# bharatlytics/faceRecognition_InfrenceEngine

Hardware: AMD Instinct MI355X
Metric: faces/sec end-to-end @1080p (higher is better)
Workload: dtype f16

## Files before the change

facerecognition_infrenceengine_amd/_lib.py:

```python
import ctypes as C
import struct
import os
import threading

_HERE = os.path.dirname(os.path.abspath(__file__))
LIB_PATH = os.path.join(_HERE, "csrc", "libfrhip.so")

_lock = threading.Lock()
_lib = None
ABI_VERSION = 104


class FrError(RuntimeError):
    pass


class ConvArgs(C.Structure):
    _fields_ = [("x", C.c_void_p), ("w", C.c_void_p), ("y", C.c_void_p),
                ("bias", C.c_void_p), ("slope", C.c_void_p), ("residual", C.c_void_p),
                ("out_f32_partial", C.c_void_p),
                ("B", C.c_int), ("H", C.c_int), ("W", C.c_int), ("Cin", C.c_int), ("Cout", C.c_int),
                ("KH", C.c_int), ("KW", C.c_int), ("stride", C.c_int), ("pad", C.c_int),
                ("Ho", C.c_int), ("Wo", C.c_int), ("bias_mode", C.c_int), ("splitk", C.c_int),
                ("x2", C.c_void_p), ("C2", C.c_int)]


class ConvStep(C.Structure):
    _fields_ = [("kind", C.c_int), ("args", ConvArgs)]


class ConvF8Args(C.Structure):
    _fields_ = [("x8", C.c_void_p), ("w8", C.c_void_p), ("y16", C.c_void_p), ("y8", C.c_void_p),
                ("oscale", C.c_void_p), ("bias", C.c_void_p), ("slope", C.c_void_p), ("residual", C.c_void_p),
                ("B", C.c_int), ("H", C.c_int), ("W", C.c_int), ("Cin", C.c_int), ("Cout", C.c_int),
                ("bias_mode", C.c_int), ("y8_mul", C.c_float), ("y8_sub", C.c_void_p)]


class RolePtr(C.c_void_p):
    role = None


class PnetLevel(C.Structure):
    _fields_ = [("x1", C.c_void_p), ("head", C.c_void_p), ("workspace", C.c_void_p), ("H1", C.c_int), ("W1", C.c_int),
# ... 50 lines not shown
    "fr_conv_walk64_weight_bytes": (_Z, [_I]),
    "fr_conv_walk64_pack": (_I, [_P, _P, _I, _P]),
    "fr_conv_walk64_f16": (_I, [_P, _P, _P, _P, _I, _P, _P, _I, _I, _I, _P]),
    "fr_conv_stage28_weight_bytes": (_Z, [_I]),
    "fr_conv_stage28_pack": (_I, [_P, _P, _P]),
    "fr_conv_stage28_f16": (_I, [_P, _P, _P, _P, _I, _I, _P]),
    "fr_conv_stage14_f8_weight_bytes": (_Z, [_I]),
    "fr_conv_stage14_f8_param_floats": (_Z, []),
    "fr_conv_stage14_f8_pack": (_I, [_P, _P, _P]),
    "fr_conv_stage14_f8": (_I, [_P, _P, _P, _P, _P, _I, _I, _P]),
    "fr_conv_splitk_epilogue": (_I, [_P, _I, _I, _I, _I, _I, _P, _I, _P, _P, _P, _P]),
    "fr_fc_reduce_l2norm": (_I, [_P, _I, _I, _I, _P, _P, _P, _P]),
    "fr_warp_affine_5pt": (_I, [_P, _I, _I, _I, _P, _P, _P, _I, _I, _P, _P, _P, _P]),
    "fr_warp_affine_5pt_slots": (_I, [_P, _I, _I, _I, _P, _P, _I, _I, _P, _P]),
    "fr_pyramid_resize_norm": (_I, [_P, _I, _I, _I, _I, _I, _P, _P]),
    "fr_dconv_f32": (_I, [_P, _P, _P, _P, _P, _I, _I, _I, _I, _I, _I, _I, _I, _I, _P, _P, _I, _P]),
    "fr_dconv_mfma_f32": (_I, [_I, _P, _P, _P, _P, _P, _I, _I, _I, _P, _P, _P, _I, _I, _P, _I, _P, _P]),
    "fr_crop_conv1_f32": (_I, [_I, _P, _I, _I, _I, _P, _P, _I, _P, _P, _P, _P, _P]),
    "fr_crop_conv1_split": (_I, [_I, _P, _I, _I, _I, _P, _P, _I, _P, _P, _P, _P, _I, _P]),
    "fr_crop_conv1_list_f32": (_I, [_I, _P, _I, _I, _I, _P, _I, _P, _P, _I, _P, _P, _P, _P, _P]),
    "fr_ro_conv2_split": (_I, [_I, _P, _P, _P, _P, _P, _I, _P, _I, _P, _P]),
    "fr_ro_gemm_weight_bytes": (_Z, [_I]),
    "fr_ro_gemm_pack": (_I, [_I, _P, _P, _P]),
    "fr_ro_gemm_split": (_I, [_I, _P, _P, _P, _P, _P, _I, _P, _I, _P]),
    "fr_ro_margin_list": (_I, [_P, _I, _P, _I, _I, _F, _F, _P, _P, _I, _P]),
    "fr_ro_scatter_rows": (_I, [_P, _P, _P, _I, _I, _P, _P]),
    "fr_pnet23_workspace_bytes": (_Z, [_I, _I, _I]),
    "fr_pnet23_split_f16": (_I, [_P, _P, _I, _I, _I, _P, _P, _P, _P, _P, _P, _P, _P, _P, _I, _F, _F, _P, _P, _Z, _P]),
    "fr_maxpool_f32": (_I, [_P, _P, _I, _I, _I, _I, _I, _I, _P]),
    "fr_pnet_conv1_band": (_I, [_I, _P, _I, _I, _I, _I, _I, _P, _P, _P, _P, _P, _P, _P, _I, _P]),
    "fr_pnet_band_tiles_count": (_Z, [_I, _I, _I]),
    "fr_pnet_band_tiles": (_I, [_P, _I, _I, _I, _P, _P, _P]),
    "fr_pnet_finish_levels": (_I, [C.POINTER(PnetLevel), _I, _I, _P, _P, _P, _P, _P, _P, _P, _P, _F, _I, _F, _P, _P]),
    "fr_pnet_pyramid_conv1": (_I, [_I, _P, _I, _I, _I, C.POINTER(PnetLevel), _I, _P, _P, _P, _P, _P, _I, _P]),
    "fr_pnet_pyramid_p23": (_I, [C.POINTER(PnetLevel), _I, _I, _P, _P, _P, _P, _P, _P, _P, _P, _I, _F, _F, _P]),
    "fr_pnet_pyramid_band_tiles": (_I, [C.POINTER(PnetLevel), _I, _I, _P, _P, _P]),
    "fr_pnet_candidates": (_I, [_P, _I, _I, _I, _F, _F, _I, _P, _P, _P, _P, _P, _P, _P, _F, _P]),
    "fr_sort_nms": (_I, [_P, _P, _P, _I, _P, _I, _I, _I, _I, _F, _I, _I, _P, _P, _P, _P, _I, _P]),
    "fr_box_refine": (_I, [_P, _P, _I, _P, _I, _I, _I, _P]),
    "fr_crop_resize_norm": (_I, [_P, _I, _I, _I, _P, _P, _I, _I, _P, _P]),
    "fr_stage_select": (_I, [_P, _P, _I, _P, _I, _I, _F, _P, _P, _P, _I, _P, _P, _P]),
    "fr_detect_sequence": (_I, [C.POINTER(Call), _I]),
}

_NOCHECK = ("fr_version", "fr_device_count")


def _slot(v, t):
    if t is _F:
        return struct.unpack("<I", struct.pack("<f", float(v)))[0]
    if t is _P:
        if v is None:
            return 0
        return int(v.value or 0) if isinstance(v, C.c_void_p) else int(v)
    return int(v) & 0xFFFFFFFFFFFFFFFF


class Lib:

    def __init__(self, cdll):
        self._c = cdll
        self._calls = {}
        self._rec = threading.local()
        for name, (res, args) in SIGNATURES.items():
            fn = getattr(cdll, name)
            fn.restype = res
# ... 91 lines not shown
```

facerecognition_infrenceengine_amd/csrc/detect_ops.hip:

```cpp
#include "detect_math.h"

__global__ void pyramid_resize_norm(const uint8_t* __restrict__ frames, int N, int H, int W, int hs, int ws,
                                    float* __restrict__ out) {
    int64_t t = (int64_t)blockIdx.x * blockDim.x + threadIdx.x;
    int64_t total = (int64_t)N * hs * ws;
    if (t >= total) return;
    int x = (int)(t % ws);
    int y = (int)((t / ws) % hs);
    int n = (int)(t / ((int64_t)ws * hs));
    const float ry = (float)H / (float)hs, rx = (float)W / (float)ws;
    Lerp ly = lerp_coord(y, ry, H), lx = lerp_coord(x, rx, W);
    const uint8_t* f = frames + (int64_t)n * H * W * 3;
    const uint8_t* r0 = f + (int64_t)ly.i0 * W * 3;
    const uint8_t* r1 = f + (int64_t)ly.i1 * W * 3;
    float* o = out + t * 3;
#pragma unroll
    for (int c = 0; c < 3; ++c) {
        int ci = 2 - c;
        float v = bilerp((float)r0[lx.i0 * 3 + ci], (float)r0[lx.i1 * 3 + ci], (float)r1[lx.i0 * 3 + ci],
                         (float)r1[lx.i1 * 3 + ci], lx.w, ly.w);
        o[c] = (v - 127.5f) * 0.0078125f;
    }
}

// ... 260 lines not shown
    const int cell = b * 256 + threadIdx.x;
    bool pass = false;
    float p = 0.f;
    const float* h = t.head[l] + ((int64_t)f * cells + (cell < cells ? cell : 0)) * 6;
    if (cell < cells && dl_may_pass(t.dl[l][(int64_t)f * cells + cell], dl_min)) {
        p = softmax2_face(h[0], h[1]);
        pass = p >= thr;
    }
    const int lane = threadIdx.x & 63, wv = threadIdx.x >> 6;
    unsigned long long m = __ballot(pass);
    if (lane == 0) wsum[wv] = __popcll(m);
    __syncthreads();
    int woff = 0;
    for (int i = 0; i < wv; ++i) woff += wsum[i];
    const int rank = base + woff + __popcll(m & ((1ull << lane) - 1ull));
    if (pass && rank < cap) {
        const int cy = cell / wc, cx = cell - cy * wc;
        const int64_t o = (int64_t)f * cap + rank;
        float4 bx;
        bx.x = floorf((2.0f * (float)cx + 1.0f) / scale);
        bx.y = floorf((2.0f * (float)cy + 1.0f) / scale);
        bx.z = floorf((2.0f * (float)cx + 12.0f) / scale);
        bx.w = floorf((2.0f * (float)cy + 12.0f) / scale);
        *reinterpret_cast<float4*>(t.boxes[l] + o * 4) = bx;
        t.scores[l][o] = p;
        *reinterpret_cast<float4*>(t.regs[l] + o * 4) = make_float4(h[2], h[3], h[4], h[5]);
    }
    if (b == nb - 1 && threadIdx.x == 0) {
        int total = base + wsum[0] + wsum[1] + wsum[2] + wsum[3];
        t.counts[l][f] = total < cap ? total : cap;
    }
}

int fr_pnet_candidates_levels_launch(const fr_pnet_level* lv, int nlevels, int nframes, float thr, int cap, float dl_min, hipStream_t s) {
    PCandLevels t;
    t.nlevels = nlevels;
    int total = 0;
    for (int l = 0; l < nlevels; ++l) {
        const int hc = lv[l].H1 - 4, wc = lv[l].W1 - 4;
        t.head[l] = lv[l].head; t.dl[l] = reinterpret_cast<const float*>(lv[l].workspace);
        t.boxes[l] = lv[l].boxes; t.scores[l] = lv[l].scores; t.regs[l] = lv[l].regs; t.counts[l] = lv[l].counts;
        t.block_counts[l] = lv[l].block_counts;
        t.cells[l] = hc * wc; t.wc[l] = wc; t.scale[l] = lv[l].scale;
        t.first[l] = total;
        total += fr_cdiv(hc * wc, 256);
    }
    t.first[nlevels] = total;
    dim3 grid(total, nframes);
    pnet_count_levels<<<grid, 256, 0, s>>>(t, thr, dl_min);
    FR_CHECK_LAUNCH("pnet_count_levels");
    pnet_emit_levels<<<grid, 256, 0, s>>>(t, thr, cap, dl_min);
    FR_CHECK_LAUNCH("pnet_emit_levels");
    return FR_OK;
}

extern "C" int fr_pnet_candidates(const float* head, int nframes, int hc, int wc, float scale, float thr, int cap,
                                  float* boxes, float* scores, float* regs, int32_t* counts, int32_t* block_counts,
                                  float* prob_out, const float* dl, float dl_min, fr_stream_t stream) {
    FR_REQUIRE(head && boxes && scores && regs && counts && block_counts, "fr_pnet_candidates: null pointer");
    FR_REQUIRE(nframes > 0 && hc > 0 && wc > 0 && cap > 0 && scale > 0.f, "fr_pnet_candidates: bad argument");
    const int cells = hc * wc;
    dim3 grid(fr_cdiv(cells, 256), nframes);
    hipStream_t s = fr_stream(stream);
    pnet_count<<<grid, 256, 0, s>>>(head, cells, thr, block_counts, prob_out, dl, dl_min);
    FR_CHECK_LAUNCH("pnet_count");
    pnet_emit<<<grid, 256, 0, s>>>(head, cells, wc, scale, thr, cap, block_counts, boxes, scores, regs, counts, dl, dl_min);
    FR_CHECK_LAUNCH("pnet_emit");
    return FR_OK;
}

__global__ void box_refine(float* __restrict__ boxes, const float* __restrict__ aux, int naux,
                           const int32_t* __restrict__ counts, int L, int cap, int mode) {
    int t = blockIdx.x * blockDim.x + threadIdx.x;
    if (t >= L * cap) return;
    int l = t / cap, i = t - l * cap;
    if (i >= counts[l]) return;
    float4 b = *reinterpret_cast<float4*>(boxes + (int64_t)t * 4);
    const float* r = aux + (int64_t)t * naux;
    float add = mode == 0 ? 0.0f : 1.0f;
    float w = b.z - b.x + add, h = b.w - b.y + add;
    float x1 = b.x + r[0] * w, y1 = b.y + r[1] * h, x2 = b.z + r[2] * w, y2 = b.w + r[3] * h;
    if (mode != 2) {
        float hh = y2 - y1, ww = x2 - x1;
        float l2 = fmaxf(ww, hh);
        x1 = x1 + ww * 0.5f - l2 * 0.5f;
        y1 = y1 + hh * 0.5f - l2 * 0.5f;
// ... 141 lines not shown
```

facerecognition_infrenceengine_amd/csrc/pnet_fused.hip:

```cpp
#include "detect_math.h"

#define P23_RH 8
#define P23_RW 32
#define P23_X1W (P23_RW + 4)
#define P23_X1PX ((P23_RH + 4) * P23_X1W)
#define P23_X2W (P23_RW + 2)
#define P23_X2PX ((P23_RH + 2) * P23_X2W)
#define P23_X2T ((P23_X2PX + 15) / 16)
#define P23_NT 512
#define P23_X1PL (448 * 32)
#define P23_X2PL (P23_X2PX * 32)

struct P23Args {
    const float* x1;
    const unsigned char* x1s;
    unsigned x1s_bytes;
    const float* w2; const float* b2; const float* s2;
    const float* w3; const float* b3; const float* s3;
    const float* hw; const float* hb;
    float* head;
    float* dl;
    int all_heads;
    int* list; int* counts; int seg_cap;
    float logit_thr;
// ... 384 lines not shown
    P23Args a;
    a.x1 = x1; a.x1s = (const unsigned char*)x1s; a.x1s_bytes = (unsigned)((int64_t)B * H1 * W1 * 64); a.w2 = w2; a.b2 = b2; a.s2 = s2; a.w3 = w3; a.b3 = b3; a.s3 = s3; a.hw = hw; a.hb = hb; a.head = head; a.all_heads = all_heads & 1;
    a.B = B; a.H1 = H1; a.W1 = W1; a.H3 = H1 - 4; a.W3 = W1 - 4;
    a.tiles_x = (a.W3 + P23_RW - 1) / P23_RW; a.tiles_y = (a.H3 + P23_RH - 1) / P23_RH;
    long long ncell, nt; int grid, seg_cap;
    p23_layout(B, H1, W1, ncell, nt, grid, seg_cap);
    FR_REQUIRE(nt < (1ll << 31) && ncell < (1ll << 31), "fr_pnet23_split_f16: too many tiles");
    const size_t need = fr_pnet23_workspace_bytes(B, H1, W1);
    FR_REQUIRE(workspace && workspace_bytes >= need, "fr_pnet23_split_f16: workspace needs %zu bytes (fr_pnet23_workspace_bytes)", need);
    a.dl = reinterpret_cast<float*>(workspace);
    a.counts = reinterpret_cast<int*>(a.dl + ncell);
    a.list = a.counts + 512;
    a.seg_cap = seg_cap;
    a.logit_thr = refine_logit_thr;
    a.band_hi = refine_band_hi;
    a.ntiles = (int)nt;
    constexpr size_t lds = (size_t)2 * P23_X1PL + (size_t)2 * P23_X2PL + 30 * 1024 + 108 * 4;
    static FrDevLatch latch;
    if (!fr_raise_lds(reinterpret_cast<const void*>(pnet23_split_f16), lds, latch)) { fr_set_error("fr_pnet23_split_f16: cannot raise dynamic LDS"); return FR_E_LAUNCH; }
    hipStream_t s = fr_stream(stream);
    pnet23_split_f16<<<grid, P23_NT, lds, s>>>(a);
    FR_CHECK_LAUNCH("pnet23_split_f16");
    if (all_heads & 2) return FR_OK;
    PRefArgs r;
    r.x1 = x1; r.w2 = w2; r.b2 = b2; r.s2 = s2; r.w3 = w3; r.b3 = b3; r.s3 = s3; r.hw = hw; r.hb = hb; r.head = head;
    r.list = a.list; r.counts = a.counts; r.seg_cap = seg_cap;
    r.B = B; r.H1 = H1; r.W1 = W1; r.H3 = a.H3; r.W3 = a.W3; r.counter = refined_count;
    pnet_refine_mfma<<<grid, 256, 0, s>>>(r);
    FR_CHECK_LAUNCH("pnet_refine_mfma");
    return FR_OK;
}

int fr_pnet_candidates_levels_launch(const fr_pnet_level* lv, int nlevels, int nframes, float thr, int cap, float dl_min, hipStream_t s);

extern "C" int fr_pnet_finish_levels(const fr_pnet_level* levels, int nlevels, int nframes, const float* w2, const float* b2,
                                     const float* s2, const float* w3, const float* b3, const float* s3, const float* hw,
                                     const float* hb, float thr, int cap, float dl_min, int32_t* refined_count, fr_stream_t stream) {
    FR_REQUIRE(levels && nlevels > 0 && nlevels <= PREF_MAXL && nframes > 0 && cap > 0, "fr_pnet_finish_levels: 1 .. %d levels", PREF_MAXL);
    FR_REQUIRE(w2 && b2 && s2 && w3 && b3 && s3 && hw && hb, "fr_pnet_finish_levels: null pointer");
    PRefLevels t;
    t.nlevels = nlevels;
    int total = 0;
    for (int l = 0; l < nlevels; ++l) {
        const fr_pnet_level& L = levels[l];
        FR_REQUIRE(L.x1 && L.head && L.workspace && L.boxes && L.scores && L.regs && L.counts && L.block_counts && L.H1 >= 5 && L.W1 >= 5 && L.scale > 0.f,
                   "fr_pnet_finish_levels: level %d: bad entry", l);
        long long ncell, nt; int grid, seg_cap;
        p23_layout(nframes, L.H1, L.W1, ncell, nt, grid, seg_cap);
        float* dl = reinterpret_cast<float*>(L.workspace);
        const int* counts = reinterpret_cast<const int*>(dl + ncell);
        t.x1[l] = L.x1; t.head[l] = L.head; t.counts[l] = counts; t.list[l] = counts + 512;
        t.seg_cap[l] = seg_cap; t.H1[l] = L.H1; t.W1[l] = L.W1;
        t.first[l] = total;
        total += grid;
    }
    t.first[nlevels] = total;
    PRefArgs r;
    r.x1 = nullptr; r.w2 = w2; r.b2 = b2; r.s2 = s2; r.w3 = w3; r.b3 = b3; r.s3 = s3; r.hw = hw; r.hb = hb; r.head = nullptr;
    r.list = nullptr; r.counts = nullptr; r.seg_cap = 0; r.B = nframes; r.H1 = r.W1 = r.H3 = r.W3 = 0; r.counter = refined_count;
    hipStream_t s = fr_stream(stream);
    pnet_refine_levels<<<total, 256, 0, s>>>(r, t);
    FR_CHECK_LAUNCH("pnet_refine_levels");
    return fr_pnet_candidates_levels_launch(levels, nlevels, nframes, thr, cap, dl_min, s);
}

__global__ __launch_bounds__(256) void pnet_band_tiles_kernel(const int* __restrict__ list, const int* __restrict__ counts, int seg_cap,
                                                             int H3, int W3, int regions_x, int regions_y, int32_t* __restrict__ tbuf,
                                                             int32_t* __restrict__ tiles) {
    const int n_list = counts[blockIdx.x];
    const int* lst = list + (size_t)blockIdx.x * seg_cap;
    const int hw3 = H3 * W3;
    for (int i = threadIdx.x; i < n_list; i += 256) {
        const int c = lst[i];
        const int n = c / hw3, r = c - n * hw3, y = r / W3, x = r - y * W3;
        const int ry0 = (2 * y) >> 4, ry1 = min((2 * y + 9) >> 4, regions_y - 1);
        const int rx0 = (2 * x) >> 6, rx1 = min((2 * x + 9) >> 6, regions_x - 1);
        for (int ry = ry0; ry <= ry1; ++ry)
            for (int rx = rx0; rx <= rx1; ++rx) {
                const int t = (n * regions_y + ry) * regions_x + rx;
                const unsigned bit = 1u << (t & 31);
                const unsigned old = atomicOr(reinterpret_cast<unsigned*>(tbuf) + 1 + (t >> 5), bit);
                if (!(old & bit)) tiles[atomicAdd(tbuf, 1)] = t;
            }
    }
}

extern "C" size_t fr_pnet_band_tiles_count(int B, int H1, int W1) {
    if (B <= 0 || H1 < 5 || W1 < 5) return 0;
    return (size_t)B * ((H1 + 7) / 8) * ((W1 + 31) / 32);
}

extern "C" int fr_pnet_band_tiles(const void* workspace, int B, int H1, int W1, int32_t* tbuf, int32_t* tiles, fr_stream_t stream) {
    FR_REQUIRE(workspace && tbuf && tiles && B > 0 && H1 >= 5 && W1 >= 5, "fr_pnet_band_tiles: bad argument");
    long long ncell, nt; int grid, seg_cap;
    p23_layout(B, H1, W1, ncell, nt, grid, seg_cap);
    const float* dl = reinterpret_cast<const float*>(workspace);
// ... 102 lines not shown
```

facerecognition_infrenceengine_amd/mtcnn.py:

```python
import contextlib
import ctypes
import logging
import math
import threading

import torch

from . import _lib


def pyramid_scales(h, w, minsize=20, factor=0.709):
    m = 12.0 / minsize
    minl = min(h, w) * m
    scales, k = [], 0
    while minl >= 12:
        scales.append(m * factor ** k)
        minl *= factor
        k += 1
    return scales


def _pool_out(n, k, s):
    o = -(-(n - k) // s) + 1
    if (o - 1) * s >= n:
# ... 115 lines not shown
        self.lib = _lib.load()
        self.device = torch.device(device)
        self.minsize, self.factor, self.thresholds = minsize, factor, tuple(float(t) for t in thresholds)
        self.cap_scale, self.keep_scale, self.cap_p, self.cap_r, self.cap_o = cap_scale, keep_scale, cap_p, cap_r, cap_o
        assert cap_scale <= 4096 and cap_p <= 1024 and cap_r <= 1024 and cap_o <= 1024
        self._sides = {}
        self._tls = threading.local()
        self.one_stream = False
        self.level_streams = 2
        self.single_frame_level_streams = self.SINGLE_FRAME_LEVEL_STREAMS
        self.phase_marks = None
        self.merged_level_nms = True
        self.batch_min_pixels = 22_000_000 if batch_min_pixels is None else int(batch_min_pixels)
        self.solo_max_frames = 7
        d = self.device
        p, r, o = ({k: v.detach().float().cpu() for k, v in s.items()} for s in (pstate, rstate, ostate))
        if canonical:
            p, r, o = (canonical_scale(s, n) for s, n in ((p, "pnet"), (r, "rnet"), (o, "onet")))
        self.p1 = _MConv(0, p["conv1.weight"], p["conv1.bias"], p["prelu1.weight"], d)
        self.p2 = _MConv(1, p["conv2.weight"], p["conv2.bias"], p["prelu2.weight"], d)
        hw = torch.cat([p["conv4_1.weight"].reshape(2, 32), p["conv4_2.weight"].reshape(4, 32)])
        hb = torch.cat([p["conv4_1.bias"], p["conv4_2.bias"]])
        self.p3 = _MConv(2, p["conv3.weight"], p["conv3.bias"], p["prelu3.weight"], d, head=(hw, hb))
        self.fused_pnet = bool(fused_pnet)
        w2p = torch.zeros((16, 10, 16)); w2p[:, :9, :10] = p["conv2.weight"].permute(0, 2, 3, 1).reshape(16, 9, 10)
        w3p = torch.zeros((32, 10, 16)); w3p[:, :9, :16] = p["conv3.weight"].permute(0, 2, 3, 1).reshape(32, 9, 16)
        self._p23 = tuple(t.to(torch.float32).contiguous().to(d) for t in (
            w2p, p["conv2.bias"], p["prelu2.weight"], w3p, p["conv3.bias"], p["prelu3.weight"], hw.t().contiguous(), hb))
        self.refine_margin = 2e-3
        self.pnet_band = True
        self.split_pconv1 = True
        self.split_pconv1_min_px = 10000
        self.pyramid_launch = True
        self.level_tensors = None
        self.refined_cells = None
        self.p23_all_heads = False
        self.use_sequence = True
        self.fused_crop = True
        self._rc1 = tuple(t.to(torch.float32).contiguous().to(d) for t in (
            r["conv1.weight"].permute(2, 3, 1, 0).reshape(27, 28), r["conv1.bias"], r["prelu1.weight"]))
        self._oc1 = tuple(t.to(torch.float32).contiguous().to(d) for t in (
            o["conv1.weight"].permute(2, 3, 1, 0).reshape(27, 32), o["conv1.bias"], o["prelu1.weight"]))
        self.split_ro = True
        self.split_conv1 = True
        self.split_tail = True
        self.ro_margin = 1e-3
        self.ro_list_cap = (1024, 256)
        def c2w(w):
            o, c = w.shape[0], w.shape[1]
            wp = torch.zeros((o, 9, 32))
            wp[:, :, :c] = w.permute(0, 2, 3, 1).reshape(o, 9, c)
            return wp
        self._rc2 = tuple(t.to(torch.float32).contiguous().to(d) for t in (c2w(r["conv2.weight"]), r["conv2.bias"], r["prelu2.weight"]))
        self._oc2 = tuple(t.to(torch.float32).contiguous().to(d) for t in (c2w(o["conv2.weight"]), o["conv2.bias"], o["prelu2.weight"]))
        self.r1 = _MConv(10, r["conv1.weight"], r["conv1.bias"], r["prelu1.weight"], d)
        self.r2 = _MConv(11, r["conv2.weight"], r["conv2.bias"], r["prelu2.weight"], d)
        self.r3 = _MConv(12, r["conv3.weight"], r["conv3.bias"], r["prelu3.weight"], d)
        self.r4 = _MConv(13, _dense_as_conv(r["dense4.weight"], 3, 64), r["dense4.bias"], r["prelu4.weight"], d)
        self.r5 = _MConv(14, torch.cat([r["dense5_1.weight"], r["dense5_2.weight"]]).reshape(6, 128, 1, 1),
                         torch.cat([r["dense5_1.bias"], r["dense5_2.bias"]]), None, d)
        self.o1 = _MConv(20, o["conv1.weight"], o["conv1.bias"], o["prelu1.weight"], d)
        self.o2 = _MConv(21, o["conv2.weight"], o["conv2.bias"], o["prelu2.weight"], d)
        self.o3 = _MConv(22, o["conv3.weight"], o["conv3.bias"], o["prelu3.weight"], d)
        self.o4 = _MConv(23, o["conv4.weight"], o["conv4.bias"], o["prelu4.weight"], d)
        self.o5 = _MConv(24, _dense_as_conv(o["dense5.weight"], 3, 128), o["dense5.bias"], o["prelu5.weight"], d)
        self._gemm = {}
# ... 150 lines not shown
        if self.fused_pnet and not getattr(self, "_unfused_logged", False):
            self._unfused_logged = True
            logging.getLogger(__name__).warning("MTCNNHIP: a %d x %d pyramid level of %d frame(s) exceeds the fused P-Net's 32-bit map "
                                                "offsets; it runs layer by layer (f32)", hs, ws, N)
        if path is not None:
            path["unfused_levels"] += 1
        self._dl = (None, 0.0)
        x, h, w = self._dconv(None, self.p1, N, hs, ws, frames=frames)
        x, h, w = self._dconv(x, self.p2, N, h, w)
        head, h, w = self._dconv(x, self.p3, N, h, w)
        return head, h, w

    def _pyramid_levels(self, N, H, W, scales):
        out = []
        for s in scales:
            hs, ws = int(math.ceil(H * s)), int(math.ceil(W * s))
            out.append((hs, ws) + tuple(self.p1.out_hw(hs, ws)))
        return out

    def _pnet_pyramid(self, frames, scales, geo, cand):
        N, H, W, _ = frames.shape
        lib, p1, path, nlev = self.lib, self.p1, self._tls.path, len(scales)
        t0, cap, lb, ls, lr, lc = cand
        lt = math.log(t0 / (1.0 - t0))
        band = self.pnet_band
        lv = (_lib.PnetLevel * nlev)()
        keep, ntile, words = [], 0, 0
        for li, (s, (hs, ws, h, w)) in enumerate(zip(scales, geo)):
            f16 = bool(band and self.split_pconv1 and h * w >= self.split_pconv1_min_px)
            xs = self._new((N, h, w, 64), torch.uint8)
            x = self._f32(N, h, w, 12)
            head = self._f32(N, h - 4, w - 4, 6)
            wsp = self._new((lib.fr_pnet23_workspace_bytes(N, h, w) // 4,), torch.float32)
            bc = self._i32(N * (-(-(h - 4) * (w - 4) // 256)))
            lv[li] = _lib.PnetLevel(x.data_ptr(), head.data_ptr(), wsp.data_ptr(), h, w, float(s), lb[li].data_ptr(), ls[li].data_ptr(),
                                    lr[li].data_ptr(), lc[li].data_ptr(), bc.data_ptr(), xs.data_ptr(), hs, ws, int(f16))
            keep.append(dict(h=h, w=w, f16=f16, x=x, xs=xs, head=head, wsp=wsp, bc=bc))
            if f16:
                nt = lib.fr_pnet_band_tiles_count(N, h, w)
                ntile, words = ntile + nt, words + (nt + 31) // 32
                path["pconv1_mfma_levels"].append((h, w))
        path["fused_levels"] += nlev
        path["band_levels"] += nlev if band else 0
        p23 = [_lib.ptr(t) for t in self._p23]
        lib.fr_pnet_pyramid_conv1(0, self._fptr(frames), N, H, W, lv, nlev, _lib.ptr(p1.w), _lib.ptr(p1.b), _lib.ptr(p1.slope),
                                  None, None, 0, self._s)
        lib.fr_pnet_pyramid_p23(lv, nlev, N, *p23, 1 if self.p23_all_heads else 0, lt - self.refine_margin,
                                lt + self.refine_margin if band else float("-inf"), self._s)
        if ntile:
            tbuf, tiles = self._i32(1 + words), self._i32(ntile)
            lib.fr_pnet_pyramid_band_tiles(lv, nlev, N, _lib.ptr(tbuf), _lib.ptr(tiles), self._s)
            lib.fr_pnet_pyramid_conv1(1, self._fptr(frames), N, H, W, lv, nlev, _lib.ptr(p1.w), _lib.ptr(p1.b), _lib.ptr(p1.slope),
                                      _lib.ptr(tiles), _lib.ptr(tbuf), ntile, self._s)
            keep[0].update(tbuf=tbuf, tiles=tiles)
        lib.fr_pnet_finish_levels(lv, nlev, N, *p23, t0, cap, lt - self.refine_margin, _lib.ptr(self.refined_cells), self._s)
        if self.level_tensors is not None:
            self.level_tensors.extend(keep)

    def crop_conv1(self, net, frames, boxes, counts, cap):
        N, H, W, _ = frames.shape
        w, b, s = self._rc1 if net == 0 else self._oc1
        p, c = (11, 28) if net == 0 else (23, 32)
        y = self._f32(N * cap, p, p, c)
        self.lib.fr_crop_conv1_f32(net, self._fptr(frames), N, H, W, _lib.ptr(boxes), _lib.ptr(counts), cap, _lib.ptr(w),
                                   _lib.ptr(b), _lib.ptr(s), _lib.ptr(y), self._s)
        return y

    def crop_conv12_split(self, net, frames, boxes, counts, cap):
        N, H, W, _ = frames.shape
        w1, b1, s1 = self._rc1 if net == 0 else self._oc1
        w2, b2, s2 = self._rc2 if net == 0 else self._oc2
        p1, p2, c2 = (11, 4, 48) if net == 0 else (23, 10, 64)
        xs = self._new((N * cap, p1 * p1, 128), torch.uint8)
        self.lib.fr_crop_conv1_split(net, self._fptr(frames), N, H, W, _lib.ptr(boxes), _lib.ptr(counts), cap, _lib.ptr(w1),
                                     _lib.ptr(b1), _lib.ptr(s1), _lib.ptr(xs), 1 if self.split_conv1 else 0, self._s)
        y = self._f32(N * cap, p2, p2, c2)
        lc = self._i32(1)
        self.lib.fr_ro_conv2_split(net, _lib.ptr(xs), _lib.ptr(w2), _lib.ptr(b2), _lib.ptr(s2), _lib.ptr(y), N * cap,
                                   _lib.ptr(counts), cap, _lib.ptr(lc), self._s)
        return y, lc

    def exact_pass(self, net, frames, boxes, counts, cap, head, thr, lc):
        N, H, W, _ = frames.shape
        w1, b1, s1 = self._rc1 if net == 0 else self._oc1
        lcap = self.ro_list_cap[net]
        nh = head.shape[1]
        lst = self._i32(lcap)
        self.lib.fr_ro_margin_list(_lib.ptr(head), nh, _lib.ptr(counts), N, cap, math.log(thr / (1.0 - thr)), self.ro_margin,
# ... 325 lines not shown
```

include/frhip.h:

```cpp
#ifndef FRHIP_H
#define FRHIP_H
#include <stddef.h>
#include <stdint.h>
#ifdef __cplusplus
extern "C" {
#endif

#define FR_OK 0
#define FR_E_INVALID (-1)
#define FR_E_LAUNCH (-2)
#define FR_E_NODEVICE (-3)

typedef void* fr_stream_t;

#define FR_ABI_VERSION 104
int fr_version(void);
const char* fr_last_error_string(void);
int fr_device_count(void);

int fr_l2norm_rows_f32(const float* x, float* out, int rows, int dim, fr_stream_t stream);

size_t fr_gallery_match_workspace(int F, int64_t N);
int fr_gallery_match_f32(const float* Q, const float* G, int F, int64_t N, int D,
                         int64_t row_offset, int64_t* out_idx, float* out_score,
                         void* workspace, size_t workspace_bytes, const int32_t* seg_counts, int seg_len,
                         fr_stream_t stream);
int fr_gallery_match_view_f32(const float* Q, const float* G, const int64_t* view, int F, int64_t Nview, int D,
                              int64_t* out_idx, float* out_score, void* workspace, size_t workspace_bytes,
                              fr_stream_t stream);
int fr_gallery_update_rows_f32(float* G, const int64_t* slots, const float* rows, int n, int D, int normalise,
                               fr_stream_t stream);
#define FR_TOPK 4
#define FR_TOPK8 8
#define FR_F8_SCALE 256.0f
size_t fr_gallery_match_f16_workspace(int F, int64_t N);
int fr_gallery_match_f16(const float* Q, const void* G16, const float* G32, int F, int64_t N, int D,
                         int64_t row_offset, int64_t* out_idx, float* out_score,
                         void* workspace, size_t workspace_bytes, const int32_t* seg_counts, int seg_len,
                         fr_stream_t stream);
size_t fr_gallery_match_f8_workspace(int F, int64_t N);
int fr_gallery_match_f8(const float* Q, const void* G8, const float* G32, int F, int64_t N, int D,
                        int64_t row_offset, int64_t* out_idx, float* out_score,
                        void* workspace, size_t workspace_bytes, const int32_t* seg_counts, int seg_len,
                        fr_stream_t stream);
#define FR_TOPK_MAX 16
size_t fr_gallery_topk_workspace(int F, int64_t N, int K);
int fr_gallery_topk_f32(const float* Q, const float* G, int F, int64_t N, int D, int K, int64_t row_offset,
                        int64_t* out_idx , float* out_score , void* workspace,
// ... 118 lines not shown
                   fr_stream_t stream);
int fr_pnet_candidates(const float* head, int nframes, int hc, int wc, float scale, float thr, int cap,
                       float* boxes, float* scores, float* regs, int32_t* counts,
                       int32_t* block_counts, float* prob_out, const float* dl, float dl_min, fr_stream_t stream);
int fr_sort_nms(const float* boxes, const float* scores, const float* aux, int naux,
                const int32_t* counts, int L, int nseg, int seg_cap, int seg_major, float thr, int mode,
                int max_keep,
                float* boxes_out, float* scores_out, float* aux_out, int32_t* counts_out,
                int cap_out, fr_stream_t stream);
int fr_box_refine(float* boxes, const float* aux, int naux, const int32_t* counts, int L, int cap,
                  int mode, fr_stream_t stream);
int fr_crop_resize_norm(const uint8_t* frames, int nframes, int H, int W, const float* boxes,
                        const int32_t* counts, int cap, int size, float* out, fr_stream_t stream);
int fr_stage_select(const float* boxes, const float* head, int nh, const int32_t* counts, int L, int cap,
                    float thr, float* boxes_out, float* scores_out, float* aux_out, int naux,
                    int32_t* counts_out, float* prob_out, fr_stream_t stream);

int fr_pnet_conv1_band(int mode, const uint8_t* frames, int B, int FH, int FW, int H, int W, const float* w, const float* bias,
                       const float* slope, float* y, void* y_split, const int32_t* list, const int32_t* list_count, int list_cap,
                       fr_stream_t stream);
size_t fr_pnet_band_tiles_count(int B, int H1, int W1);
int fr_pnet_band_tiles(const void* workspace, int B, int H1, int W1, int32_t* tbuf, int32_t* tiles, fr_stream_t stream);
typedef struct {
    const float* x1; float* head; void* workspace;
    int H1, W1; float scale;
    float* boxes; float* scores; float* regs; int32_t* counts; int32_t* block_counts;
    void* x1s;
    int hs, ws;
    int f16;
} fr_pnet_level;
int fr_pnet_finish_levels(const fr_pnet_level* levels, int nlevels, int nframes, const float* w2, const float* b2,
                          const float* s2, const float* w3, const float* b3, const float* s3, const float* hw,
                          const float* hb, float thr, int cap, float dl_min, int32_t* refined_count, fr_stream_t stream);
int fr_pnet_pyramid_conv1(int mode, const uint8_t* frames, int B, int FH, int FW, const fr_pnet_level* levels, int nlevels,
                          const float* w, const float* bias, const float* slope, const int32_t* list, const int32_t* list_count,
                          int list_cap, fr_stream_t stream);
int fr_pnet_pyramid_p23(const fr_pnet_level* levels, int nlevels, int nframes, const float* w2, const float* b2, const float* s2,
                        const float* w3, const float* b3, const float* s3, const float* hw, const float* hb, int all_heads,
                        float refine_logit_thr, float refine_band_hi, fr_stream_t stream);
int fr_pnet_pyramid_band_tiles(const fr_pnet_level* levels, int nlevels, int nframes, int32_t* tbuf, int32_t* tiles, fr_stream_t stream);

enum { FR_FN_DCONV_MFMA = 1, FR_FN_PNET23 = 2, FR_FN_PNET_CANDIDATES = 3, FR_FN_SORT_NMS = 4, FR_FN_BOX_REFINE = 5,
       FR_FN_CROP_CONV1 = 6, FR_FN_STAGE_SELECT = 7,
       FR_FN_EVENT_RECORD = 8 , FR_FN_STREAM_WAIT = 9  };
typedef struct {
    int32_t fn; int32_t nargs;
    uint64_t a[22];
} fr_call;
int fr_detect_sequence(const fr_call* calls, int ncalls);

#ifdef __cplusplus
}
#endif
#endif
```

Before: 26270.

## Replace two-pass PNet candidate count/emit with one-pass per-level extract kernel

Adds a single kernel, one 1024-thread block per (frame, level), that scans the cells, builds ballot bitmasks in shared memory, ranks the passing cells with a block prefix sum and writes boxes, scores and regressions in order. It replaces the count kernel plus emit kernel pair and removes the block_counts buffer, cutting a launch and a global round trip. The trade is far less parallelism: one block per frame and level must scan every cell serially. The new path is enabled by default through onepass_candidates, and cap is limited to 4096.

```diff
diff --git a/facerecognition_infrenceengine_amd/_lib.py b/facerecognition_infrenceengine_amd/_lib.py
--- a/facerecognition_infrenceengine_amd/_lib.py
+++ b/facerecognition_infrenceengine_amd/_lib.py
@@ -8,7 +8,7 @@
 
 _lock = threading.Lock()
 _lib = None
-ABI_VERSION = 104
+ABI_VERSION = 105
 
 
 class FrError(RuntimeError):
@@ -125,6 +125,8 @@
     "fr_pnet_band_tiles_count": (_Z, [_I, _I, _I]),
     "fr_pnet_band_tiles": (_I, [_P, _I, _I, _I, _P, _P, _P]),
     "fr_pnet_finish_levels": (_I, [C.POINTER(PnetLevel), _I, _I, _P, _P, _P, _P, _P, _P, _P, _P, _F, _I, _F, _P, _P]),
+    "fr_pnet_extract_levels": (_I, [C.POINTER(PnetLevel), _I, _I, _F, _I, _F, _P]),
+    "fr_pnet_finish_levels_onepass": (_I, [C.POINTER(PnetLevel), _I, _I, _P, _P, _P, _P, _P, _P, _P, _P, _F, _I, _F, _P, _P]),
     "fr_pnet_pyramid_conv1": (_I, [_I, _P, _I, _I, _I, C.POINTER(PnetLevel), _I, _P, _P, _P, _P, _P, _I, _P]),
     "fr_pnet_pyramid_p23": (_I, [C.POINTER(PnetLevel), _I, _I, _P, _P, _P, _P, _P, _P, _P, _P, _I, _F, _F, _P]),
     "fr_pnet_pyramid_band_tiles": (_I, [C.POINTER(PnetLevel), _I, _I, _P, _P, _P]),
diff --git a/facerecognition_infrenceengine_amd/csrc/detect_ops.hip b/facerecognition_infrenceengine_amd/csrc/detect_ops.hip
--- a/facerecognition_infrenceengine_amd/csrc/detect_ops.hip
+++ b/facerecognition_infrenceengine_amd/csrc/detect_ops.hip
@@ -316,8 +316,7 @@
     }
 }
 
-int fr_pnet_candidates_levels_launch(const fr_pnet_level* lv, int nlevels, int nframes, float thr, int cap, float dl_min, hipStream_t s) {
-    PCandLevels t;
+static int pcand_table(PCandLevels& t, const fr_pnet_level* lv, int nlevels) {
     t.nlevels = nlevels;
     int total = 0;
     for (int l = 0; l < nlevels; ++l) {
@@ -330,12 +329,154 @@
         total += fr_cdiv(hc * wc, 256);
     }
     t.first[nlevels] = total;
+    return total;
+}
+
+int fr_pnet_candidates_levels_launch(const fr_pnet_level* lv, int nlevels, int nframes, float thr, int cap, float dl_min, hipStream_t s) {
+    PCandLevels t;
+    const int total = pcand_table(t, lv, nlevels);
     dim3 grid(total, nframes);
     pnet_count_levels<<<grid, 256, 0, s>>>(t, thr, dl_min);
     FR_CHECK_LAUNCH("pnet_count_levels");
     pnet_emit_levels<<<grid, 256, 0, s>>>(t, thr, cap, dl_min);
     FR_CHECK_LAUNCH("pnet_emit_levels");
     return FR_OK;
+}
+
+#define PEXT_NT 1024
+#define PEXT_CHUNKS 1024
+#define PEXT_MAXCAP 4096
+__device__ __forceinline__ float4 pext_load(const float* __restrict__ dl, int cell0, int cells, bool active) {
+    float4 v = make_float4(-INFINITY, -INFINITY, -INFINITY, -INFINITY);
+    if (active && cell0 + 3 >= 0 && cell0 < cells) v = *reinterpret_cast<const float4*>(dl + cell0);
+    return v;
+}
+__global__ __launch_bounds__(PEXT_NT) void pnet_extract_levels(PCandLevels t, float thr, int cap, float dl_min) {
+    const int f = blockIdx.x, l = blockIdx.y;
+    const int cells = t.cells[l], wc = t.wc[l];
+    const float scale = t.scale[l];
+    const float* __restrict__ dl = t.dl[l] + (int64_t)f * cells;
+    const float* __restrict__ head = t.head[l] + (int64_t)f * cells * 6;
+    const int lane = threadIdx.x & 63, wv = threadIdx.x >> 6;
+    const int off = (int)((reinterpret_cast<uintptr_t>(dl) >> 2) & 3);
+    const int nchunk = (cells + off + 255) >> 8;
+    __shared__ unsigned long long bits[PEXT_CHUNKS][4];
+    __shared__ int list[PEXT_MAXCAP];
+    __shared__ int wcnt[PEXT_NT / 64];
+    const unsigned long long below = (1ull << lane) - 1ull;
+    int base = 0;
+    for (int c0 = 0; c0 < nchunk; c0 += PEXT_CHUNKS) {
+        const int nc = min(PEXT_CHUNKS, nchunk - c0), per = (nc + PEXT_NT / 64 - 1) / (PEXT_NT / 64);
+        const int cb = min(wv * per, nc), ce = min(cb + per, nc);
+        const int lane0 = (c0 << 8) + 4 * lane - off;
+        int cnt = 0;
+        float4 d[4];
+#pragma unroll
+        for (int u = 0; u < 4; ++u) d[u] = pext_load(dl, lane0 + ((cb + u) << 8), cells, cb + u < ce);
+        for (int c = cb; c < ce; c += 4) {
+            float2 hh[4][4];
+            bool may[4][4];
+#pragma unroll
+            for (int u = 0; u < 4; ++u) {
+                const float du[4] = {d[u].x, d[u].y, d[u].z, d[u].w};
+#pragma unroll
+                for (int j = 0; j < 4; ++j) {
+                    const int cell = lane0 + ((c + u) << 8) + j;
+                    may[u][j] = cell >= 0 && cell < cells && c + u < ce && dl_may_pass(du[j], dl_min);
+                    hh[u][j] = make_float2(0.f, 0.f);
+                    if (may[u][j]) hh[u][j] = *reinterpret_cast<const float2*>(head + (int64_t)cell * 6);
+                }
+            }
+            float4 dn[4];
+#pragma unroll
+            for (int u = 0; u < 4; ++u) dn[u] = pext_load(dl, lane0 + ((c + 4 + u) << 8), cells, c + 4 + u < ce);
+#pragma unroll
+            for (int u = 0; u < 4; ++u) {
+                if (c + u >= ce) break;
+#pragma unroll
+                for (int j = 0; j < 4; ++j) {
+                    unsigned long long m = 0;
+                    if (__ballot(may[u][j])) {
+                        const bool pass = may[u][j] && softmax2_face(hh[u][j].x, hh[u][j].y) >= thr;
+                        m = __ballot(pass);
+                    }
+                    if (lane == 0) bits[c + u][j] = m;
+                    cnt += __popcll(m);
+                }
+            }
+#pragma unroll
+            for (int u = 0; u < 4; ++u) d[u] = dn[u];
+        }
+        if (lane == 0) wcnt[wv] = cnt;
+        __syncthreads();
+        int wbase = base, total = 0;
+        for (int i = 0; i < PEXT_NT / 64; ++i) {
+            const int n = wcnt[i];
+            if (i < wv) wbase += n;
+            total += n;
+        }
+        for (int c = cb; c < ce && wbase < cap; ++c) {
+            const unsigned long long m0 = bits[c][0], m1 = bits[c][1], m2 = bits[c][2], m3 = bits[c][3];
+            if (!(m0 | m1 | m2 | m3)) continue;
+            const unsigned long long m[4] = {m0, m1, m2, m3};
+            int rank = wbase + __popcll(m0 & below) + __popcll(m1 & below) + __popcll(m2 & below) + __popcll(m3 & below);
+#pragma unroll
+            for (int j = 0; j < 4; ++j) {
+                if (!((m[j] >> lane) & 1ull)) continue;
+                if (rank < cap) list[rank] = lane0 + (c << 8) + j;
+                ++rank;
+            }
+            wbase += __popcll(m0) + __popcll(m1) + __popcll(m2) + __popcll(m3);
+        }
+        __syncthreads();
+        const int end = min(base + total, cap);
+        for (int rank = base + (int)threadIdx.x; rank < end; rank += PEXT_NT) {
+            const int cell = list[rank];
+            const float* h = head + (int64_t)cell * 6;
+            const float2 h01 = *reinterpret_cast<const float2*>(h), h23 = *reinterpret_cast<const float2*>(h + 2),
+                         h45 = *reinterpret_cast<const float2*>(h + 4);
+            const float p = softmax2_face(h01.x, h01.y);
+            const int cy = cell / wc, cx = cell - cy * wc;
+            const int64_t o = (int64_t)f * cap + rank;
+            float4 bx;
+            bx.x = floorf((2.0f * (float)cx + 1.0f) / scale);
+            bx.y = floorf((2.0f * (float)cy + 1.0f) / scale);
+            bx.z = floorf((2.0f * (float)cx + 12.0f) / scale);
+            bx.w = floorf((2.0f * (float)cy + 12.0f) / scale);
+            *reinterpret_cast<float4*>(t.boxes[l] + o * 4) = bx;
+            t.scores[l][o] = p;
+            *reinterpret_cast<float4*>(t.regs[l] + o * 4) = make_float4(h23.x, h23.y, h45.x, h45.y);
+        }
+        base += total;
+        if (base >= cap) break;
+        __syncthreads();
+    }
+    if (threadIdx.x == 0) t.counts[l][f] = base < cap ? base : cap;
+}
+
+int fr_pnet_extract_levels_launch(const fr_pnet_level* lv, int nlevels, int nframes, float thr, int cap, float dl_min, hipStream_t s) {
+    FR_REQUIRE(cap <= PEXT_MAXCAP, "pnet_extract_levels: cap %d above the %d slots of its cell list", cap, PEXT_MAXCAP);
+    for (int l = 0; l < nlevels; ++l)
+        FR_REQUIRE((reinterpret_cast<uintptr_t>(lv[l].workspace) & 15) == 0 && (reinterpret_cast<uintptr_t>(lv[l].boxes) & 15) == 0 &&
+                   (reinterpret_cast<uintptr_t>(lv[l].head) & 7) == 0 &&
+                   (reinterpret_cast<uintptr_t>(lv[l].regs) & 15) == 0 && (int64_t)(lv[l].H1 - 4) * (lv[l].W1 - 4) < (1 << 30),
+                   "pnet_extract_levels: level %d: misaligned pointer or too many cells", l);
+    PCandLevels t;
+    pcand_table(t, lv, nlevels);
+    pnet_extract_levels<<<dim3(nframes, nlevels), PEXT_NT, 0, s>>>(t, thr, cap, dl_min);
+    FR_CHECK_LAUNCH("pnet_extract_levels");
+    return FR_OK;
+}
+
+extern "C" int fr_pnet_extract_levels(const fr_pnet_level* levels, int nlevels, int nframes, float thr, int cap, float dl_min,
+                                      fr_stream_t stream) {
+    FR_REQUIRE(levels && nlevels > 0 && nlevels <= PCAND_MAXL && nframes > 0 && cap > 0, "fr_pnet_extract_levels: 1 .. %d levels", PCAND_MAXL);
+    for (int l = 0; l < nlevels; ++l) {
+        const fr_pnet_level& L = levels[l];
+        FR_REQUIRE(L.head && L.workspace && L.boxes && L.scores && L.regs && L.counts && L.H1 >= 5 && L.W1 >= 5 && L.scale > 0.f,
+                   "fr_pnet_extract_levels: level %d: bad entry", l);
+    }
+    return fr_pnet_extract_levels_launch(levels, nlevels, nframes, thr, cap, dl_min, fr_stream(stream));
 }
 
 extern "C" int fr_pnet_candidates(const float* head, int nframes, int hc, int wc, float scale, float thr, int cap,
diff --git a/facerecognition_infrenceengine_amd/csrc/pnet_fused.hip b/facerecognition_infrenceengine_amd/csrc/pnet_fused.hip
--- a/facerecognition_infrenceengine_amd/csrc/pnet_fused.hip
+++ b/facerecognition_infrenceengine_amd/csrc/pnet_fused.hip
@@ -440,10 +440,11 @@
 }
 
 int fr_pnet_candidates_levels_launch(const fr_pnet_level* lv, int nlevels, int nframes, float thr, int cap, float dl_min, hipStream_t s);
-
-extern "C" int fr_pnet_finish_levels(const fr_pnet_level* levels, int nlevels, int nframes, const float* w2, const float* b2,
-                                     const float* s2, const float* w3, const float* b3, const float* s3, const float* hw,
-                                     const float* hb, float thr, int cap, float dl_min, int32_t* refined_count, fr_stream_t stream) {
+int fr_pnet_extract_levels_launch(const fr_pnet_level* lv, int nlevels, int nframes, float thr, int cap, float dl_min, hipStream_t s);
+
+static int pnet_finish_levels(bool onepass, const fr_pnet_level* levels, int nlevels, int nframes, const float* w2, const float* b2,
+                              const float* s2, const float* w3, const float* b3, const float* s3, const float* hw,
+                              const float* hb, float thr, int cap, float dl_min, int32_t* refined_count, fr_stream_t stream) {
     FR_REQUIRE(levels && nlevels > 0 && nlevels <= PREF_MAXL && nframes > 0 && cap > 0, "fr_pnet_finish_levels: 1 .. %d levels", PREF_MAXL);
     FR_REQUIRE(w2 && b2 && s2 && w3 && b3 && s3 && hw && hb, "fr_pnet_finish_levels: null pointer");
     PRefLevels t;
@@ -451,7 +452,7 @@
     int total = 0;
     for (int l = 0; l < nlevels; ++l) {
         const fr_pnet_level& L = levels[l];
-        FR_REQUIRE(L.x1 && L.head && L.workspace && L.boxes && L.scores && L.regs && L.counts && L.block_counts && L.H1 >= 5 && L.W1 >= 5 && L.scale > 0.f,
+        FR_REQUIRE(L.x1 && L.head && L.workspace && L.boxes && L.scores && L.regs && L.counts && (onepass || L.block_counts) && L.H1 >= 5 && L.W1 >= 5 && L.scale > 0.f,
                    "fr_pnet_finish_levels: level %d: bad entry", l);
         long long ncell, nt; int grid, seg_cap;
         p23_layout(nframes, L.H1, L.W1, ncell, nt, grid, seg_cap);
@@ -469,7 +470,20 @@
     hipStream_t s = fr_stream(stream);
     pnet_refine_levels<<<total, 256, 0, s>>>(r, t);
     FR_CHECK_LAUNCH("pnet_refine_levels");
-    return fr_pnet_candidates_levels_launch(levels, nlevels, nframes, thr, cap, dl_min, s);
+    return onepass ? fr_pnet_extract_levels_launch(levels, nlevels, nframes, thr, cap, dl_min, s)
+                   : fr_pnet_candidates_levels_launch(levels, nlevels, nframes, thr, cap, dl_min, s);
+}
+
+extern "C" int fr_pnet_finish_levels(const fr_pnet_level* levels, int nlevels, int nframes, const float* w2, const float* b2,
+                                     const float* s2, const float* w3, const float* b3, const float* s3, const float* hw,
+                                     const float* hb, float thr, int cap, float dl_min, int32_t* refined_count, fr_stream_t stream) {
+    return pnet_finish_levels(false, levels, nlevels, nframes, w2, b2, s2, w3, b3, s3, hw, hb, thr, cap, dl_min, refined_count, stream);
+}
+
+extern "C" int fr_pnet_finish_levels_onepass(const fr_pnet_level* levels, int nlevels, int nframes, const float* w2, const float* b2,
+                                             const float* s2, const float* w3, const float* b3, const float* s3, const float* hw,
+                                             const float* hb, float thr, int cap, float dl_min, int32_t* refined_count, fr_stream_t stream) {
+    return pnet_finish_levels(true, levels, nlevels, nframes, w2, b2, s2, w3, b3, s3, hw, hb, thr, cap, dl_min, refined_count, stream);
 }
 
 __global__ __launch_bounds__(256) void pnet_band_tiles_kernel(const int* __restrict__ list, const int* __restrict__ counts, int seg_cap,
diff --git a/facerecognition_infrenceengine_amd/mtcnn.py b/facerecognition_infrenceengine_amd/mtcnn.py
--- a/facerecognition_infrenceengine_amd/mtcnn.py
+++ b/facerecognition_infrenceengine_amd/mtcnn.py
@@ -171,6 +171,7 @@
         self.split_pconv1 = True
         self.split_pconv1_min_px = 10000
         self.pyramid_launch = True
+        self.onepass_candidates = True
         self.level_tensors = None
         self.refined_cells = None
         self.p23_all_heads = False
@@ -387,9 +388,10 @@
             x = self._f32(N, h, w, 12)
             head = self._f32(N, h - 4, w - 4, 6)
             wsp = self._new((lib.fr_pnet23_workspace_bytes(N, h, w) // 4,), torch.float32)
-            bc = self._i32(N * (-(-(h - 4) * (w - 4) // 256)))
+            bc = None if self.onepass_candidates else self._i32(N * (-(-(h - 4) * (w - 4) // 256)))
             lv[li] = _lib.PnetLevel(x.data_ptr(), head.data_ptr(), wsp.data_ptr(), h, w, float(s), lb[li].data_ptr(), ls[li].data_ptr(),
-                                    lr[li].data_ptr(), lc[li].data_ptr(), bc.data_ptr(), xs.data_ptr(), hs, ws, int(f16))
+                                    lr[li].data_ptr(), lc[li].data_ptr(), bc.data_ptr() if bc is not None else None, xs.data_ptr(),
+                                    hs, ws, int(f16))
             keep.append(dict(h=h, w=w, f16=f16, x=x, xs=xs, head=head, wsp=wsp, bc=bc))
             if f16:
                 nt = lib.fr_pnet_band_tiles_count(N, h, w)
@@ -408,7 +410,8 @@
             lib.fr_pnet_pyramid_conv1(1, self._fptr(frames), N, H, W, lv, nlev, _lib.ptr(p1.w), _lib.ptr(p1.b), _lib.ptr(p1.slope),
                                       _lib.ptr(tiles), _lib.ptr(tbuf), ntile, self._s)
             keep[0].update(tbuf=tbuf, tiles=tiles)
-        lib.fr_pnet_finish_levels(lv, nlev, N, *p23, t0, cap, lt - self.refine_margin, _lib.ptr(self.refined_cells), self._s)
+        finish = lib.fr_pnet_finish_levels_onepass if self.onepass_candidates else lib.fr_pnet_finish_levels
+        finish(lv, nlev, N, *p23, t0, cap, lt - self.refine_margin, _lib.ptr(self.refined_cells), self._s)
         if self.level_tensors is not None:
             self.level_tensors.extend(keep)
 
diff --git a/include/frhip.h b/include/frhip.h
--- a/include/frhip.h
+++ b/include/frhip.h
@@ -13,7 +13,7 @@
 
 typedef void* fr_stream_t;
 
-#define FR_ABI_VERSION 104
+#define FR_ABI_VERSION 105
 int fr_version(void);
 const char* fr_last_error_string(void);
 int fr_device_count(void);
@@ -198,6 +198,10 @@
 int fr_pnet_finish_levels(const fr_pnet_level* levels, int nlevels, int nframes, const float* w2, const float* b2,
                           const float* s2, const float* w3, const float* b3, const float* s3, const float* hw,
                           const float* hb, float thr, int cap, float dl_min, int32_t* refined_count, fr_stream_t stream);
+int fr_pnet_extract_levels(const fr_pnet_level* levels, int nlevels, int nframes, float thr, int cap, float dl_min, fr_stream_t stream);
+int fr_pnet_finish_levels_onepass(const fr_pnet_level* levels, int nlevels, int nframes, const float* w2, const float* b2,
+                                  const float* s2, const float* w3, const float* b3, const float* s3, const float* hw,
+                                  const float* hb, float thr, int cap, float dl_min, int32_t* refined_count, fr_stream_t stream);
 int fr_pnet_pyramid_conv1(int mode, const uint8_t* frames, int B, int FH, int FW, const fr_pnet_level* levels, int nlevels,
                           const float* w, const float* bias, const float* slope, const int32_t* list, const int32_t* list_count,
                           int list_cap, fr_stream_t stream);
```

Result: slower. 25640 (-2.4%).
